# citibeth/spsparse

Hardware: AMD Instinct MI355X
Metric: nnz(C)/s for C=A*A SpGEMM (higher is better)
Workload: dtype f64

## Files before the change

### spsparse_amd/csrc/capi.hip

```cpp
#include "internal.h"

#include <cstdio>
#include <cstdlib>
#include <cstring>
#include <algorithm>
#include <exception>
#include <vector>

using namespace spsamd;

#define API_GUARD(ctx, ...)                                                         \
	if ((ctx)->busy) { (ctx)->last_error = "context busy: a streamed multiply is delivering on it"; return SPSAMD_EINVAL; } \
	try { __VA_ARGS__ }                                                             \
	catch (const spsamd::Error &e) { (ctx)->last_error = e.msg; return e.code; }    \
	catch (const std::bad_alloc &) { (ctx)->last_error = "host allocation failed"; return SPSAMD_ENOMEM; } \
	catch (const std::exception &e) { (ctx)->last_error = e.what(); return SPSAMD_EINVAL; }

extern "C" const char *spsamd_version(void) { return "spsparse_amd 0.2 (gfx950)"; }

extern "C" int spsamd_ctx_create(spsamd_ctx **out, int device, void *hip_stream)
{
	if (!out) return SPSAMD_EINVAL;
	*out = nullptr;
	int ndev = 0;
// ... 223 lines not shown
			SPS_HIP(hipMemcpyAsync(vv, V->val, V->nnz * sizeof(double), kind, c->stream));
			fill_zero(c, vz, V->nnz * sizeof(int32_t));
			Vm.idx0 = vi; Vm.idx1 = vz; Vm.val = vv;
		}
		int rc = multiply_body(c, C, scalei, A, transpose_A, scalej, &Vm, '.', nullptr, duplicate_policy, zero_nan,
			sink_kind, sink_flags & ~SPSAMD_SINK_PERMUTE, res, "V", true, nullptr, true);
		res->shape1 = 0;
		res->idx1 = nullptr;
		return rc;
	)
}


struct spsamd_operand {
	spsamd::Prepared p;
	uint64_t shape0 = 0, shape1 = 0;
};

extern "C" int spsamd_operand_prepare(spsamd_ctx *c, const spsamd_coo *X, char transpose, int role, int duplicate_policy, int zero_nan,
	spsamd_operand **out)
{
	if (!c) return SPSAMD_EINVAL;
	API_GUARD(c,
		if (!X || !out) throw Error{SPSAMD_EINVAL, "null operand or result"};
		*out = nullptr;
		if (role != SPSAMD_AS_A && role != SPSAMD_AS_B && role != (SPSAMD_AS_A | SPSAMD_AS_B)) throw Error{SPSAMD_EINVAL, "bad role"};
		if (duplicate_policy < 0 || duplicate_policy > 2) throw Error{SPSAMD_EINVAL, "bad duplicate_policy"};
		if (X->mem == SPSAMD_MEM_PREPARED) throw Error{SPSAMD_EINVAL, "the operand is a prepared one already"};
		if (zero_nan && role == (SPSAMD_AS_A | SPSAMD_AS_B))
			throw Error{SPSAMD_EINVAL, "under zero_nan the two sides of a product drop different NaNs (multiply_sparse.hpp:167-168): prepare one operand per side"};
		SPS_HIP(hipSetDevice(c->device));
		c->arena.reset();
		const int lead = transpose == 'T' ? 1 : 0;
		const int ref_lead = (role & SPSAMD_AS_A) ? lead : 1 - lead;
		ConMat m;
		consolidate_operand(c, X, lead, ref_lead, duplicate_policy, zero_nan, &m);
		spsamd_operand *h = new spsamd_operand();
		struct Guard { spsamd_operand *h; ~Guard() { if (h) { h->p.release(); delete h; } } } guard{h};
		h->shape0 = X->shape0; h->shape1 = X->shape1;
		Prepared &p = h->p;
		p.ctx = c; p.owns = true; p.lead = lead;
		p.m = m;
		const size_t n = m.nnz;
		size_t want = (n + 64) * (16 + 12 + 8) + (m.nrow + 66) * 4 + 65536;
		uint32_t maxlen = 0;
		if (n) {
			Prepared view;
			view.ctx = c; view.m = m;
			prepared_row_structure(c, &view);
			maxlen = view.maxlen;
		}
		if ((role & SPSAMD_AS_B) && maxlen > 64) {
			const uint64_t W = m.ncol > (uint64_t(1) << 21) ? 16384 : 8192, nwin = (m.ncol + W - 1) / W, nwp = (nwin + 7) & ~7ull, nrowb = m.nrow + 1;
			const uint64_t idx = nrowb * (nwin + 1) * 4 + nrowb * nwp * 2 + (nrowb * nwin + 1) * 4 + (n + 8) * 12 + 8192;
			size_t freeb = 0, totalb = 0;
			if (idx <= 64 * (uint64_t)n * 16 && hipMemGetInfo(&freeb, &totalb) == hipSuccess && idx + want < freeb / 2) want += idx;
		}
		p.reserve(want);
		p.m.row = p.get<int32_t>(n ? n : 1); p.m.col = p.get<int32_t>(n ? n : 1); p.m.val = p.get<double>(n ? n : 1);
		if (n) {
			SPS_HIP(hipMemcpyAsync(p.m.row, m.row, n * sizeof(int32_t), hipMemcpyDeviceToDevice, c->stream));
			SPS_HIP(hipMemcpyAsync(p.m.col, m.col, n * sizeof(int32_t), hipMemcpyDeviceToDevice, c->stream));
			SPS_HIP(hipMemcpyAsync(p.m.val, m.val, n * sizeof(double), hipMemcpyDeviceToDevice, c->stream));
		}
		prepared_row_structure(c, &p);
		SPS_HIP(hipStreamSynchronize(c->stream));
		guard.h = nullptr;
		*out = h;
		return SPSAMD_OK;
	)
}

extern "C" int spsamd_operand_as_coo(const spsamd_operand *h, spsamd_coo *out)
{
	if (!h || !out) return SPSAMD_EINVAL;
	out->idx0 = (const int32_t *)h; out->idx1 = nullptr; out->val = nullptr;
	out->nnz = h->p.m.nnz; out->shape0 = h->shape0; out->shape1 = h->shape1;
	out->sort0 = h->p.lead; out->mem = SPSAMD_MEM_PREPARED;
	return SPSAMD_OK;
}

extern "C" uint64_t spsamd_operand_bytes(const spsamd_operand *h) { return h ? h->p.owned_bytes : 0; }

extern "C" void spsamd_operand_destroy(spsamd_operand *h)
{
	if (!h) return;
	if (h->p.ctx) { (void)hipSetDevice(h->p.ctx->device); (void)hipStreamSynchronize(h->p.ctx->stream); if (h->p.ctx->side) (void)hipStreamSynchronize(h->p.ctx->side); }
	h->p.release();
	delete h;
}

extern "C" int spsamd_result_fetch(spsamd_ctx *c, const spsamd_result *res, spsamd_chunk_fn cb, void *user)
{
	if (!c) return SPSAMD_EINVAL;
	API_GUARD(c,
		if (!res || !cb) throw Error{SPSAMD_EINVAL, "null result or callback"};
		if (res->nnz == 0) return SPSAMD_OK;
		if (!res->idx0 || !res->val) throw Error{SPSAMD_EINVAL, "result has no COO tuples (DIGEST sink?)"};
		SPS_HIP(hipSetDevice(c->device));
		const size_t chunk = size_t(1) << 20;
		char *h = (char *)c->host_staging(2 * chunk * 16);
		hipEvent_t ev[2] = {c->ev[EV_FETCH0], c->ev[EV_FETCH1]};
		auto issue = [&](uint64_t o, int b) {
			size_t n = (size_t)std::min<uint64_t>(chunk, res->nnz - o);
			char *hb = h + (size_t)b * chunk * 16;
			SPS_HIP(hipMemcpyAsync(hb, res->idx0 + o, n * 4, hipMemcpyDeviceToHost, c->stream));
			if (res->idx1) SPS_HIP(hipMemcpyAsync(hb + chunk * 4, res->idx1 + o, n * 4, hipMemcpyDeviceToHost, c->stream));
// ... 315 lines not shown
```

### spsparse_amd/csrc/internal.h

```cpp
#pragma once

#include <hip/hip_runtime.h>
#include <stdint.h>
#include <stddef.h>
#include <string>
#include <vector>

#include "../../include/spsparse_amd.h"

namespace spsamd {


struct Error {
	int code;
	std::string msg;
};

#define SPS_HIP(call)                                                              \
	do {                                                                           \
		hipError_t e_ = (call);                                                    \
		if (e_ != hipSuccess)                                                      \
			throw ::spsamd::Error{SPSAMD_EHIP, std::string(#call) + ": " + hipGetErrorString(e_)}; \
	} while (0)

// ... 264 lines not shown

void first_kept_key_raw(spsamd_ctx *c, const spsamd_coo *Xdev, int lead, int ref_lead, unsigned long long *out_dev);

uint32_t inspect_operand(spsamd_ctx *c, const int32_t *major, const int32_t *minor, const double *val, size_t n,
	uint64_t nrow, uint64_t ncol);

struct RowList {
	uint32_t *beg = nullptr;
	int32_t *id = nullptr;
	uint32_t nrows = 0;
};
void dim_beginnings(spsamd_ctx *c, const ConMat &m, RowList *out);
void dim_beginnings(spsamd_ctx *c, const ConMat &m, const uint32_t *ptr, RowList *out);

uint32_t *sorted_permutation(spsamd_ctx *c, const spsamd_coo *X, int lead);

uint32_t *dense_rowptr(spsamd_ctx *c, const ConMat &m, uint32_t extra, uint32_t *into = nullptr);

struct __attribute__((packed, aligned(4))) BTup { int32_t col; uint32_t vlo, vhi; };

struct SolveSchedule {
	bool built = false;
	uint32_t levels = 0, max_level_rows = 0;
	uint64_t tuples_used = 0;
	int64_t zero_pivot = -1;
	uint32_t *level_ptr = nullptr;
	uint32_t *rows = nullptr;
	std::vector<uint32_t> h_level_ptr, h_level_max;
	bool have_work = false;
	std::vector<uint32_t> h_level_work;
};

struct Prepared {
	spsamd_ctx *ctx = nullptr;
	ConMat m;
	int lead = 0;
	bool owns = false;
	std::vector<void *> owned;
	uint64_t owned_bytes = 0;
	char *slab = nullptr;
	size_t slab_left = 0;
	void reserve(size_t bytes);
	uint32_t *rowptr = nullptr;
	uint32_t maxlen = 0;
	bool have_maxlen = false;
	RowList rl;
	bool have_rl = false;
	BTup *btup = nullptr;
	int W = 0;
	uint32_t nwin = 0, nwp = 0;
	uint64_t nrowb = 0;
	uint32_t *bwin = nullptr;
	uint16_t *wcnt = nullptr;
	uint32_t *wptr = nullptr;
	BTup *btw = nullptr;
	SolveSchedule solve[2][2];
	void *alloc(size_t bytes);
	template <class T> T *get(size_t n) { return (T *)alloc(n * sizeof(T)); }
	void release();
};


struct ScaleDev {
	bool present = false;
	int32_t *pos = nullptr;
	const double *val = nullptr;
	uint64_t dim = 0;
};

void upload_scale(spsamd_ctx *c, const spsamd_vec *s, uint64_t dim, const char *name, ScaleDev *out);

struct MultiplyArgs {
	double C;
	ScaleDev si, sj, sk;
	ConMat A, B;
	int sink_kind, sink_flags;
	Prepared *pa = nullptr, *pb = nullptr;
	hipEvent_t b_ready = nullptr;
	OutSet *out = nullptr;
	bool static_walk = false;
};
void spgemm(spsamd_ctx *c, MultiplyArgs &a, spsamd_result *res);
void prepared_row_structure(spsamd_ctx *c, Prepared *p);
BTup *prepared_btup(spsamd_ctx *c, Prepared *p);

struct OperandParts { Prepared *pa = nullptr, *pb = nullptr; hipEvent_t b_ready = nullptr; };
int multiply_body(spsamd_ctx *c, double C,
	const spsamd_vec *scalei, const spsamd_coo *A, char transpose_A,
	const spsamd_vec *scalej, const spsamd_coo *B, char transpose_B,
	const spsamd_vec *scalek, int duplicate_policy, int zero_nan,
	int sink_kind, int sink_flags, spsamd_result *res, const char *what, bool arena_ready, const OperandParts *parts = nullptr, bool b_rank1 = false);


int multiply_stream(spsamd_ctx *c, double C,
	const spsamd_vec *scalei, const spsamd_coo *A, char transpose_A,
	const spsamd_vec *scalej, const spsamd_coo *B, char transpose_B,
	const spsamd_vec *scalek, int duplicate_policy, int zero_nan,
	int sink_flags, size_t block_tuples, spsamd_chunk_fn cb, void *user,
	spsamd_result *res, spsamd_stream_stats *stats);


struct DenseOperand {
	const uint32_t *rowptr = nullptr;
	const BTup *tup = nullptr;
	uint64_t nrow = 0, ncol = 0;
	uint32_t nnz = 0;
// ... 155 lines not shown
```

### spsparse_amd/csrc/k_hash.hip

```cpp
#include "spgemm_host.h"
#include "spgemm_hash.h"

namespace spsamd {

template <int T, int NT, int MODE, bool WINDOWED, bool PAT>
__global__ __launch_bounds__(NT) void k_hash(const Cell *cells, uint32_t ncell, const uint32_t *xb, RowMeta m,
	const uint32_t *bwin, uint32_t nwin1, EmitParams ep, SinkParams sk)
{
	__shared__ int32_t h_key[T];
	__shared__ double h_val[MODE == MODE_COUNT ? 1 : T];
	__shared__ uint16_t occ[T / 2];
	__shared__ uint64_t s_sort[MODE == MODE_STORE ? T / 2 : 1];
	__shared__ uint16_t s_cnt[MODE == MODE_STORE ? 16 * ((T / 2 + NT - 1) / NT) * (NT / 64) : 1];
	__shared__ Expand<NT, T / 2> X;
	__shared__ uint32_t scr32[NT / 64 + 1];
	__shared__ uint32_t s_nocc;
	__shared__ PatCell s_pat;
	__shared__ unsigned long long s_u64[2 * (NT / 64)];
	__shared__ double s_f64[NT / 64];

	const unsigned tid = threadIdx.x;
	for (int q = tid; q < T; q += NT) { h_key[q] = -1; if (MODE != MODE_COUNT) h_val[q] = 0.0; }
	PatAcc pat; pat_init(pat);
	if (tid == 0) pat_reset(&s_pat);
	DigestAcc dacc{0, 0, 0.0};
	uint32_t flip = 0;

	const CellWalk walk = cell_walk(xb, ncell);
	const uint32_t stride = walk.stride, cend = walk.end;
	const bool any_cell = walk.first < cend;
	const uint32_t clast = any_cell ? cend - 1 : 0;
	const uint32_t zlane = cell_pend_zero();
	Cell rec1 = cells[min(walk.first, clast)];
	CellPend pend2 = cell_pend_load(cells, min(walk.first + stride, clast), zlane);
	uint32_t nlo, nlen; double na;
	{
		const uint32_t e = rec1.beg + tid;
		const bool act = e < rec1.end;
		const uint32_t ec = act ? e : rec1.beg;
		const int32_t k = m.acol[ec];
		uint32_t lo, hi;
		if (WINDOWED) { const uint32_t *bw = bwin + (uint64_t)k * nwin1; lo = bw[rec1.wa]; hi = bw[rec1.wb]; }
		else { lo = m.bptr[k]; hi = m.bptr[k + 1]; }
		na = m.aval[ec];
		nlo = lo; nlen = act ? hi - lo : 0u;
	}
	for (uint32_t ci = walk.first; ci < cend; ci += stride) {
		const Cell cell = rec1;
		const uint32_t beg = cell.beg, end = cell.end, wa = cell.wa, wb = cell.wb, seg = cell.seg;
		const int32_t rowid = cell.rowid;
		const uint32_t lo0 = nlo, len0 = nlen; const double a0 = na;
		rec1 = cell_from_pend(pend2);
		pend2 = cell_pend_load(cells, min(ci + 2 * stride, clast), zlane);
		const uint32_t ne = rec1.beg + tid;
		const bool nact = (ci + stride < cend) && ne < rec1.end;
		const uint32_t nec = ne < rec1.end ? ne : rec1.beg;
		const int32_t nk = m.acol[nec];
		na = m.aval[nec];
		const bool oversize = cell.prods > (uint32_t)(T / 2);
		if (oversize && tid == 0) atomicOr(sk.err, 1u);
		lds_barrier();
		if (tid == 0) s_nocc = 0;

		for (uint32_t chunk = beg; chunk < (oversize ? beg : end); chunk += NT) {
			uint32_t lo = lo0, len = len0; double a = a0;
			if (chunk != beg) {
				uint32_t e = chunk + tid;
				lo = 0; len = 0; a = 0;
				if (e < end) {
					int32_t k = m.acol[e];
					if (WINDOWED) { const uint32_t *bw = bwin + (uint64_t)k * nwin1; lo = bw[wa]; len = bw[wb] - lo; }
					else { lo = m.bptr[k]; len = m.bptr[k + 1] - lo; }
					a = m.aval[e];
				}
			}
			uint32_t total, nzc, ex;
			expand_load(X, lo, len, a, &total, &nzc, flip, &ex);
			if (total == 0) continue;
			if (!ABL(ep, 4)) expand_batch(X, 0, total, nzc);
			if (ABL(ep, 1)) total = 0;
			if (ep.ordered) hash_products_ordered<T, NT, T / 2, MODE>(X, 0, nzc, m, h_key, h_val, occ, &s_nocc);
			else hash_products<T, NT, T / 2, MODE, PAT>(X, 0, total, 0, m, h_key, h_val, occ, &s_nocc, pat);
			lds_barrier();
		}
		if (PAT) pat_publish(pat, &s_pat);
		{
			uint32_t lo, hi;
			if (WINDOWED) { const uint32_t *bw = bwin + (uint64_t)nk * nwin1; lo = bw[rec1.wa]; hi = bw[rec1.wb]; }
			else { lo = m.bptr[nk]; hi = m.bptr[nk + 1]; }
			nlo = lo; nlen = nact ? hi - lo : 0u;
		}
		lds_barrier();
		uint32_t nocc = s_nocc;
		if (ABL(ep, 2)) nocc = 0;
		uint32_t colbase = 0, colbits = ep.ncolbits;
		if (WINDOWED) { colbase = wa << ep.wshift; colbits = ep.wshift + (wb - wa > 1 ? 32 - __builtin_clz(wb - wa - 1) : 0); }
		const double pthr = PAT ? pat_threshold(&s_pat, end - beg) : -1.0;
		hash_emit<T, NT, MODE, PAT>(nocc, rowid, seg, ep, sk, h_key, h_val, occ, s_sort, scr32, dacc, s_cnt, colbase, colbits, m, beg, end, pthr);
		if (PAT) { lds_barrier(); if (tid == 0) pat_reset(&s_pat); }
	}
	if (MODE == MODE_DIGEST) digest_flush<NT>(sk.digest, dacc.cnt, dacc.hash, dacc.sum, s_u64, s_f64);
}

template <int MODE>
__global__ __launch_bounds__(TILE_NT) void k_hash_tiles(const Tile *tiles, uint32_t ntile, const TCell *tcells, RowMeta m,
	const uint32_t *bwin, uint32_t nwin1, EmitParams ep, SinkParams sk)
{
	constexpr int NT = TILE_NT, T = TILE_T;
	__shared__ int32_t h_key[T];
	__shared__ double h_val[MODE == MODE_COUNT ? 1 : T];
	__shared__ uint16_t occ[T / 2];
	__shared__ uint64_t s_sort[MODE == MODE_STORE ? T / 2 : 1];
	__shared__ uint16_t s_cnt[MODE == MODE_STORE ? 16 * ((T / 2 + NT - 1) / NT) * (NT / 64) : 1];
	constexpr int PB = MODE == MODE_STORE ? TILE_PB_STORE : TILE_PB;
	__shared__ Expand<NT, PB> X;
	__shared__ uint32_t scr32[NT / 64 + 1];
	__shared__ uint32_t s_nocc;
	__shared__ PatCell s_pat;
	__shared__ uint32_t cellP[TILE_MAXCELLS + 1];
	__shared__ unsigned long long s_u64[2 * (NT / 64)];
	__shared__ double s_f64[NT / 64];

	const unsigned tid = threadIdx.x;
	for (int q = tid; q < T; q += NT) { h_key[q] = -1; if (MODE != MODE_COUNT) h_val[q] = 0.0; }
	PatAcc pat; pat_init(pat);
	if (tid == 0) pat_reset(&s_pat);
	DigestAcc dacc{0, 0, 0.0};
	uint32_t flip = 0;
	STAMP_BEGIN();
	TileWalk<BoundsRowMajor, false> walk;
	for (walk.begin(tiles, ntile, tcells, m.acol, m.aval, BoundsRowMajor{bwin, nwin1}); walk.more(); walk.next()) {
		const TileTake t = walk.take();
		const Tile &tile = t.tile;
		const uint32_t myc = tid >> t.lsh, myei = tid & ((1u << t.lsh) - 1u);

		STAMP_COUNT(8);
		STAMP(0);
		lds_barrier();
		STAMP(1);
		uint32_t total, nzc, ex;
		expand_load(X, t.lo, t.len, t.a, &total, &nzc, flip, &ex);
		if (myei == 0 && myc < tile.ncells) cellP[myc] = ex;
		if (tid == 0) { cellP[tile.ncells] = total; s_nocc = 0; }
		const uint32_t seg_of_mine = t.seg;
		STAMP(2);
		if (total) expand_batch(X, 0, total, nzc);
		else lds_barrier();
		STAMP(3);
		walk.expanded();
		for (uint32_t c = 0; c < tile.ncells; ++c) {
			STAMP_COUNT(9);
			STAMP(0);
			const uint32_t p0 = cellP[c], p1 = cellP[c + 1];
			if (ep.ordered) {
				const uint32_t q0 = expand_lookup(X, p0, 0), q1 = expand_lookup(X, p1 - 1, 0) + 1;
				hash_products_ordered<T, NT, PB, MODE>(X, q0, q1, m, h_key, h_val, occ, &s_nocc);
			} else if (ep.pattern) hash_products<T, NT, PB, MODE, true>(X, p0, p1, 0, m, h_key, h_val, occ, &s_nocc, pat);
			else hash_products<T, NT, PB, MODE, false>(X, p0, p1, 0, m, h_key, h_val, occ, &s_nocc, pat);
			if (ep.pattern) pat_publish(pat, &s_pat);
			STAMP(4);
			lds_barrier();
			STAMP(5);
			const uint32_t nocc = s_nocc;
			if (myc == c && myei == 0) scr32[NT / 64] = seg_of_mine;
			lds_barrier();
			const uint32_t seg = scr32[NT / 64];
			if (tid == 0) s_nocc = 0;
			uint32_t colbase = 0, colbits = 0;
			if (MODE == MODE_STORE) {
				const TCell tcc = tcells[tile.first + c];
				colbase = (uint32_t)tcc.wa << ep.wshift;
				colbits = ep.wshift + (tcc.wb - tcc.wa > 1 ? 32 - __builtin_clz((uint32_t)(tcc.wb - tcc.wa) - 1u) : 0);
			}
			STAMP(6);
			const double pthr = ep.pattern ? pat_threshold(&s_pat, tile.end - tile.beg) : -1.0;
			if (ep.pattern) hash_emit<T, NT, MODE, true>(nocc, tile.rowid, seg, ep, sk, h_key, h_val, occ, s_sort, scr32, dacc, s_cnt, colbase, colbits, m, tile.beg, tile.end, pthr);
			else hash_emit<T, NT, MODE, false>(nocc, tile.rowid, seg, ep, sk, h_key, h_val, occ, s_sort, scr32, dacc, s_cnt, colbase, colbits, m, tile.beg, tile.end, pthr);
			STAMP(7);
			if (ep.pattern) { lds_barrier(); if (tid == 0) pat_reset(&s_pat); }
			lds_barrier();
		}
	}
	STAMP_FLUSH();
	if (MODE == MODE_DIGEST) digest_flush<NT>(sk.digest, dacc.cnt, dacc.hash, dacc.sum, s_u64, s_f64);
}

template <int T, int NT, int MODE, bool WINDOWED>
static void launch_hash(spsamd_ctx *c, const Cell *cells, uint32_t ncell, const uint32_t *xb, const RowMeta &m, const uint32_t *bwin,
	uint32_t nwin1, const EmitParams &ep, const SinkParams &sk)
{
	if (!ncell) return;
	unsigned grid = std::min<unsigned>(ncell, (unsigned)(c->num_cu * resident_per_cu<&k_hash<T, NT, MODE, WINDOWED, false>>(NT)));
	if (grid >= 64) grid &= ~7u;
	if (ep.pattern) k_hash<T, NT, MODE, WINDOWED, true><<<dim3(grid), dim3(NT), 0, c->stream>>>(cells, ncell, xb, m, bwin, nwin1, ep, sk);
	else k_hash<T, NT, MODE, WINDOWED, false><<<dim3(grid), dim3(NT), 0, c->stream>>>(cells, ncell, xb, m, bwin, nwin1, ep, sk);
	SPS_LAUNCH_CHECK();
}

template <int MODE>
void launch_mid(spsamd_ctx *c, const Bins &b, const MidCells &mc, const RowMeta &m, const EmitParams &ep, const SinkParams &sk)
{
	launch_hash<1024, 256, MODE, false>(c, mc.cells[0], b.count[5], nullptr, m, nullptr, 0, ep, sk);
	launch_hash<4096, 512, MODE, false>(c, mc.cells[1], b.count[6], nullptr, m, nullptr, 0, ep, sk);
	launch_hash<8192, 512, MODE, false>(c, mc.cells[2], b.count[7], nullptr, m, nullptr, 0, ep, sk);
}

template <int MODE>
void launch_hash_windowed(spsamd_ctx *c, const Heavy &hv, const RowMeta &m, const EmitParams &ep, const SinkParams &sk)
{
	launch_hash<1024, 256, MODE, true>(c, hv.cells[0], hv.ncell[0], hv.xb[0], m, hv.bwin, hv.nwin1, ep, sk);
	launch_hash<3072, 512, MODE, true>(c, hv.cells[1], hv.ncell[1], hv.xb[1], m, hv.bwin, hv.nwin1, ep, sk);
	launch_hash<4096, 512, MODE, true>(c, hv.cells[2], hv.ncell[2], hv.xb[2], m, hv.bwin, hv.nwin1, ep, sk);
	launch_hash<8192, 512, MODE, true>(c, hv.cells[3], hv.ncell[3], hv.xb[3], m, hv.bwin, hv.nwin1, ep, sk);
}

template <int MODE>
void launch_tiles_v1(spsamd_ctx *c, const Heavy &hv, const RowMeta &m, const EmitParams &ep, const SinkParams &sk)
{
	const unsigned grid = std::min<unsigned>(hv.ntile, (unsigned)(c->num_cu * resident_per_cu<&k_hash_tiles<MODE>>(TILE_NT)));
	const SinkParams &sks = stamps_sink(c, sk, grid);
	k_hash_tiles<MODE><<<dim3(grid), dim3(TILE_NT), 0, c->stream>>>(hv.tb.tiles, hv.ntile, hv.tb.tcells, m, hv.bwin, hv.nwin1, ep, sks);
	SPS_LAUNCH_CHECK();
	static const char *const nm[10] = {"pre", "Bwait", "expand_load", "expand_batch", "products", "Bwait2", "segbcast", "emit", "tiles", "cells"};
	stamps_report(c, sks, grid, "k_hash_tiles", nm, 10);
}

template void launch_mid<MODE_COUNT>(spsamd_ctx *, const Bins &, const MidCells &, const RowMeta &, const EmitParams &, const SinkParams &);
template void launch_mid<MODE_STORE>(spsamd_ctx *, const Bins &, const MidCells &, const RowMeta &, const EmitParams &, const SinkParams &);
template void launch_mid<MODE_DIGEST>(spsamd_ctx *, const Bins &, const MidCells &, const RowMeta &, const EmitParams &, const SinkParams &);
template void launch_hash_windowed<MODE_COUNT>(spsamd_ctx *, const Heavy &, const RowMeta &, const EmitParams &, const SinkParams &);
template void launch_hash_windowed<MODE_STORE>(spsamd_ctx *, const Heavy &, const RowMeta &, const EmitParams &, const SinkParams &);
template void launch_hash_windowed<MODE_DIGEST>(spsamd_ctx *, const Heavy &, const RowMeta &, const EmitParams &, const SinkParams &);
template void launch_tiles_v1<MODE_COUNT>(spsamd_ctx *, const Heavy &, const RowMeta &, const EmitParams &, const SinkParams &);
template void launch_tiles_v1<MODE_STORE>(spsamd_ctx *, const Heavy &, const RowMeta &, const EmitParams &, const SinkParams &);
template void launch_tiles_v1<MODE_DIGEST>(spsamd_ctx *, const Heavy &, const RowMeta &, const EmitParams &, const SinkParams &);

#ifdef SPSAMD_ABLATIONS
void set_ablation_word(spsamd_ctx *c, int word)
{
	SPS_HIP(hipMemcpyToSymbolAsync(HIP_SYMBOL(g_abl), &word, sizeof(int), 0, hipMemcpyHostToDevice, c->stream));
	SPS_HIP(hipStreamSynchronize(c->stream));
}
#endif

}
```

### spsparse_amd/csrc/spgemm_host.h

```cpp
#pragma once
#include "spgemm_dev.h"

namespace spsamd {

struct Bins {
	uint32_t count[NBIN];
	uint32_t off[NBIN + 1];
	uint32_t *rows;
};

struct MidCells { Cell *cells[3] = {nullptr, nullptr, nullptr}; };

struct TooWide { uint64_t width; };
constexpr uint64_t COLBLK = (uint64_t)2048 << 14;

struct Heavy {
	uint32_t n = 0;
	uint64_t tuples = 0;
	uint32_t *rows = nullptr;
	uint32_t *bwin = nullptr;
	uint32_t nwin = 0, nwin1 = 0;
	uint32_t *winprod = nullptr;
	uint32_t ncell[NCLS] = {};
	Cell *cells[NCLS] = {};
	CellBases cnt{}, base{};
	uint32_t *xb[NCLS] = {};
	int W = 8192;
	uint32_t cell_cap = CELL_CAP_DEFAULT, dense_min = DENSE_MIN_DEFAULT;
	TileBases tb{};
	uint32_t ntile = 0, ntcell = 0;
	TileBases tb2{};
	uint32_t ntile2 = 0, ntcell2 = 0;
	uint32_t direct_min = 0;
	int tiles2 = 0;
	uint32_t *tile_ctr = nullptr;
	uint32_t span_cap = 0;
	uint32_t alt_cap = 0, alt_span = 0;
	unsigned long long *alt_cells = nullptr;
	uint32_t long_cap = 0, long_dense_min = 0;
	bool coo = false;
	unsigned long long clsprod[NCLS + 2] = {};
	uint32_t *wptr = nullptr;
	BTup *btw = nullptr;
	uint64_t nrowb = 0;
	uint32_t nnzb = 0;

	uint32_t narrow() const { return ((uint64_t)nnzb + DENSE_R) * 12u < (uint64_t(1) << 32) ? 1u : 0u; }
	template <int MODE> uint32_t *tile_claim() const { return tile_ctr ? tile_ctr + (MODE == MODE_STORE ? 1 : 0) : nullptr; }
};

static inline TileKinds tile_kinds(const Heavy &hv)
{
	TileKinds tk{{hv.tb, hv.tb2}, hv.direct_min, hv.span_cap, hv.long_cap, hv.long_dense_min,
		hv.tiles2 == 0 ? (uint32_t)BM_MAXOUT : (uint32_t)(TILE_T / 2), hv.alt_cap, hv.alt_span, hv.alt_cells};
	return tk;
}

static inline float elapsed(hipEvent_t a, hipEvent_t b)
{
	float ms = 0;
	SPS_HIP(hipEventElapsedTime(&ms, a, b));
	return ms;
}

template <auto KERNEL>
static inline int resident_per_cu(int nt)
{
	static int per_cu = 0;
	if (!per_cu) {
		int nb = 0;
		if (hipOccupancyMaxActiveBlocksPerMultiprocessor(&nb, KERNEL, nt, 0) != hipSuccess || nb < 1) nb = 1;
		per_cu = nb;
	}
// ... 62 lines not shown
```

### spsparse_amd/csrc/symbolic_heavy.hip

```cpp
#include "spgemm_host.h"

namespace spsamd {

__global__ void k_cell_cost(const Cell *cells, uint32_t n, uint32_t fixed, uint32_t *cost)
{
	uint32_t i = blockIdx.x * blockDim.x + threadIdx.x;
	if (i < n) cost[i] = cells[i].prods + fixed;
}

__global__ void k_xcd_bounds(const int64_t *pref, uint32_t n, uint32_t *xb)
{
	uint32_t x = threadIdx.x;
	if (x > 8) return;
	int64_t target = pref[n] / 8 * x;
	uint32_t lo = 0, hi = n;
	while (lo < hi) { uint32_t mid = lo + ((hi - lo) >> 1); if (pref[mid] < target) lo = mid + 1; else hi = mid; }
	xb[x] = x == 8 ? n : lo;
}


constexpr int BT_NT = 256;
constexpr size_t BT_LDS = 36 * 1024;

__global__ __launch_bounds__(BT_NT) void k_wcnt_count(const int32_t *brow, const int32_t *bcol, uint32_t nnzb, uint32_t wshift, uint32_t nwp, uint32_t *wcnt32)
{
	const uint32_t lane = lane_id();
	const uint32_t nchunk = (nnzb + 63u) >> 6, nwaves = gridDim.x * (BT_NT / 64);
	for (uint32_t ch = blockIdx.x * (BT_NT / 64) + wave_id(); ch < nchunk; ch += nwaves) {
		const uint32_t e = (ch << 6) + lane;
		const bool valid = e < nnzb;
		const unsigned long long key = valid ? (unsigned long long)(uint32_t)brow[e] * nwp + ((uint32_t)bcol[e] >> wshift) : ~0ull;
		const unsigned long long kprev = __shfl_up(key, 1, 64), knext = __shfl_down(key, 1, 64);
		const bool is_start = valid && (lane == 0 || key != kprev);
		const bool is_end = valid && (lane == 63 || key != knext);
		const unsigned long long sm = __ballot(is_start);
		if (is_end) {
			const unsigned long long upto = sm & (lane == 63 ? ~0ull : ((2ull << lane) - 1ull));
			const uint32_t first = 63u - (uint32_t)__clzll((long long)upto);
			atomicAdd(&wcnt32[key >> 1], (lane - first + 1u) << ((uint32_t)(key & 1ull) << 4));
		}
	}
}

__global__ __launch_bounds__(BT_NT) void k_bwin_scan(const uint16_t *wcnt, const uint32_t *bptr, uint64_t nrowb, uint32_t tr, uint32_t nwin, uint32_t nwp,
	uint32_t *bwin)
{
	extern __shared__ uint32_t s_dyn[];
	const uint32_t nwin1 = nwin + 1u, lane = lane_id(), wv = wave_id(), nph = nwp >> 1;
	const uint64_t k0 = (uint64_t)blockIdx.x * tr;
	const uint32_t rows = (uint32_t)std::min<uint64_t>(tr, nrowb - k0);
	uint32_t *s_ptr = s_dyn + (size_t)tr * nph;
	{
		const uint4 *src = reinterpret_cast<const uint4 *>(wcnt + k0 * nwp);
		uint4 *dst = reinterpret_cast<uint4 *>(s_dyn);
		for (uint32_t i = threadIdx.x; i < (rows * nph) >> 2; i += BT_NT) dst[i] = src[i];
		for (uint32_t r = threadIdx.x; r < rows; r += BT_NT) s_ptr[r] = bptr[k0 + r];
	}
	__syncthreads();
	for (uint32_t r = wv; r < rows; r += BT_NT / 64) {
		const uint32_t *src = s_dyn + r * nph;
		uint32_t carry = s_ptr[r];
		uint32_t *bw = bwin + (k0 + r) * nwin1;
		for (uint32_t c0 = 0; c0 < nwin1; c0 += 64u) {
			const uint32_t w = c0 + lane;
			const uint32_t v = w < nwin ? (src[w >> 1] >> ((w & 1u) << 4)) & 0xFFFFu : 0u;
			const uint32_t inc = wave_inclusive_scan_u32(v);
			if (w < nwin1) bw[w] = carry + inc - v;
			carry += (uint32_t)__builtin_amdgcn_readlane((int)inc, 63);
		}
	}
}

constexpr int WM_TR = 256;
constexpr int WM_CS = 72;
constexpr int WM_NT = 256;

__global__ __launch_bounds__(WM_NT) void k_wm_tile_sums(const uint16_t *wcnt, uint64_t nrowb, uint32_t nwp, uint32_t ntile, uint32_t *tilesum)
{
	extern __shared__ uint32_t s_dyn[];
	const uint32_t nq = nwp >> 3;
	for (uint32_t w = threadIdx.x; w < nwp; w += WM_NT) s_dyn[w] = 0;
	__syncthreads();
	const uint64_t k0 = (uint64_t)blockIdx.x * WM_TR;
	const uint32_t rows = (uint32_t)std::min<uint64_t>(WM_TR, nrowb - k0);
	const uint4 *tab = reinterpret_cast<const uint4 *>(wcnt + k0 * nwp);
	uint32_t acc[8] = {0, 0, 0, 0, 0, 0, 0, 0};
	uint32_t myq = 0xFFFFFFFFu;
	const uint32_t stride = (WM_NT / nq) * nq;
	if (threadIdx.x < stride) {
		myq = threadIdx.x % nq;
		for (uint32_t i = threadIdx.x; i < rows * nq; i += stride) {
			const uint4 x = tab[i];
			acc[0] += x.x & 0xFFFFu; acc[1] += x.x >> 16; acc[2] += x.y & 0xFFFFu; acc[3] += x.y >> 16;
			acc[4] += x.z & 0xFFFFu; acc[5] += x.z >> 16; acc[6] += x.w & 0xFFFFu; acc[7] += x.w >> 16;
		}
#pragma unroll
		for (int u = 0; u < 8; ++u) if (acc[u]) atomicAdd(&s_dyn[myq * 8u + u], acc[u]);
	}
	__syncthreads();
	for (uint32_t w = threadIdx.x; w < nwp; w += WM_NT) tilesum[(uint64_t)w * ntile + blockIdx.x] = s_dyn[w];
}

__global__ __launch_bounds__(WM_NT) void k_wm_tile_scan(uint32_t *tilesum, uint32_t ntile, uint32_t *wtot)
{
	__shared__ uint32_t scratch[WM_NT / 64 + 1];
	uint32_t *a = tilesum + (uint64_t)blockIdx.x * ntile;
	uint32_t carry = 0;
	for (uint32_t base = 0; base < ntile; base += WM_NT) {
		const uint32_t i = base + threadIdx.x;
		const uint32_t v = i < ntile ? a[i] : 0u;
		uint32_t tot;
		const uint32_t ex = block_exclusive_scan<uint32_t, WM_NT>(v, scratch, &tot);
		if (i < ntile) a[i] = carry + ex;
		carry += tot;
	}
	if (threadIdx.x == 0) wtot[blockIdx.x] = carry;
}

// ... 269 lines not shown
{
	uint32_t i = blockIdx.x * blockDim.x + threadIdx.x;
	if (i < n) dst[i] = src[perm[i]];
}

static void heavy_window_major(spsamd_ctx *c, Heavy &hv, const ConMat &B, uint32_t wshift, const uint16_t *wcnt, uint32_t nwp, Prepared *pb)
{
	hipStream_t st = c->stream;
	const uint64_t nrowb = hv.nrowb, total = nrowb * hv.nwin;
	const uint32_t ntile = (uint32_t)((nrowb + WM_TR - 1) / WM_TR);
	hv.wptr = pb->get<uint32_t>(total + 1);
	uint32_t *tilesum = c->arena.get<uint32_t>((uint64_t)nwp * ntile);
	uint32_t *wtot = c->arena.get<uint32_t>(hv.nwin), *wbase = c->arena.get<uint32_t>(hv.nwin);
	k_wm_tile_sums<<<dim3(ntile), dim3(WM_NT), nwp * sizeof(uint32_t), st>>>(wcnt, nrowb, nwp, ntile, tilesum);
	SPS_LAUNCH_CHECK();
	k_wm_tile_scan<<<dim3(hv.nwin), dim3(WM_NT), 0, st>>>(tilesum, ntile, wtot);
	SPS_LAUNCH_CHECK();
	k_wm_bases<<<dim3(1), dim3(WM_NT), 0, st>>>(wtot, hv.nwin, wbase, hv.wptr + total);
	SPS_LAUNCH_CHECK();
	k_wm_ptr<<<dim3(ntile), dim3(WM_NT), 0, st>>>(wcnt, nrowb, hv.nwin, nwp, ntile, tilesum, wbase, hv.wptr);
	SPS_LAUNCH_CHECK();
	hv.btw = pb->get<BTup>((size_t)B.nnz + DENSE_R);
	k_wm_scatter<<<dim3(grid_for(B.nnz)), dim3(256), 0, st>>>(B.row, B.col, B.val, B.nnz, wshift, hv.bwin, hv.nwin1, hv.wptr, nrowb, hv.btw);
	SPS_LAUNCH_CHECK();
}

int heavy_b_index(spsamd_ctx *c, const ConMat &B, const uint32_t *bptr, uint32_t extra, uint64_t nheavy, Prepared *pb)
{
	hipStream_t st = c->stream;
	int W = B.ncol > (uint64_t(1) << 21) ? 16384 : 8192;
	if (c->tune.window == 8192 || c->tune.window == 16384) W = c->tune.window;
	const uint32_t wshift = W == 8192 ? 13 : 14;
	const uint32_t nwin = (uint32_t)((B.ncol + W - 1) >> wshift);
	if (nwin > (uint32_t)WH_MAXW) throw TooWide{COLBLK};
	const uint64_t nrowb = B.nrow + extra;
	if (pb->bwin && pb->W == W && pb->nrowb == nrowb) return W;
	const uint64_t per_window = nrowb * 12u + nheavy * 4u;
	uint64_t budget;
	const uint64_t room = (pb->owns || c->arena.slabs.empty()) ? 0 : c->arena.slabs.back().cap - c->arena.slabs.back().used;
	if (c->tune.index_budget_mb > 0) budget = (uint64_t)c->tune.index_budget_mb << 20;
	else if (per_window * (nwin + 1ull) <= room) budget = room;
	else {
		size_t freeb = 0, totalb = 0;
		SPS_HIP(hipMemGetInfo(&freeb, &totalb));
		budget = (uint64_t)((double)(freeb + room) * 0.8);
	}
	if (per_window * (nwin + 1ull) > budget && nwin > 1) {
		uint64_t fit = budget / per_window;
		if (fit < 2) throw Error{SPSAMD_ENOMEM, "the window index of one column window of op(B) does not fit the device"};
		uint64_t w2 = 1;
		while (w2 * 2 <= fit - 1) w2 *= 2;
		throw TooWide{w2 << wshift};
	}
	const uint32_t nwin1 = nwin + 1, nwp = (nwin + 7u) & ~7u;
	pb->reserve(nrowb * nwin1 * 4 + nrowb * nwp * 2 + (nrowb * nwin + 1) * 4 + ((size_t)B.nnz + DENSE_R) * sizeof(BTup) + 4096);
	pb->bwin = pb->get<uint32_t>(nrowb * nwin1);
	pb->wcnt = pb->get<uint16_t>(nrowb * nwp);
	pb->W = W; pb->nwin = nwin; pb->nwp = nwp; pb->nrowb = nrowb;
	pb->wptr = nullptr; pb->btw = nullptr;
	fill_zero(c, pb->wcnt, nrowb * nwp * sizeof(uint16_t));
	k_wcnt_count<<<dim3((unsigned)c->num_cu * 16u), dim3(BT_NT), 0, st>>>(B.row, B.col, B.nnz, wshift, nwp, reinterpret_cast<uint32_t *>(pb->wcnt));
	SPS_LAUNCH_CHECK();
	uint32_t tr = 256;
	while (tr > 4 && (size_t)tr * (nwp * 2 + 4) > BT_LDS) tr >>= 1;
	static bool lds_attr = false;
	if (!lds_attr) { SPS_HIP(hipFuncSetAttribute((const void *)k_bwin_scan, hipFuncAttributeMaxDynamicSharedMemorySize, (int)BT_LDS)); lds_attr = true; }
	k_bwin_scan<<<dim3((unsigned)((nrowb + tr - 1) / tr)), dim3(BT_NT), (size_t)tr * (nwp * 2 + 4), st>>>(pb->wcnt, bptr, nrowb, tr, nwin, nwp, pb->bwin);
	SPS_LAUNCH_CHECK();
	return W;
}

void heavy_prepare(spsamd_ctx *c, Heavy &hv, const Bins &bins, const RowMeta &m, const ConMat &B, const uint32_t *bptr,
	uint32_t extra, uint32_t *nseg, bool ordered, bool pattern, Prepared *pb)
{
	hipStream_t st = c->stream;
	hv.W = heavy_b_index(c, B, bptr, extra, hv.n, pb);
	const uint32_t wshift = hv.W == 8192 ? 13 : 14;
	hv.nwin = (uint32_t)((B.ncol + hv.W - 1) >> wshift);
	hv.nwin1 = hv.nwin + 1;
	const uint64_t nrowb = B.nrow + extra;
	const bool have_wmajor = pb->wptr != nullptr;
	hv.nrowb = nrowb;
	hv.nnzb = B.nnz;
	hv.rows = bins.rows + bins.off[8];
	hv.winprod = c->arena.get<uint32_t>((uint64_t)hv.n * hv.nwin);
	const uint32_t nwp = (hv.nwin + 7u) & ~7u;
	hv.bwin = pb->bwin;
	uint16_t *wcnt = pb->wcnt;
	if (!c->tune.no_wmajor && have_wmajor) { hv.wptr = pb->wptr; hv.btw = pb->btw; }
	else if (!c->tune.no_wmajor) {
		{
			SideScope on_side(c, 0, true);
			heavy_window_major(c, hv, B, wshift, wcnt, nwp, pb);
		}
		pb->wptr = hv.wptr; pb->btw = hv.btw;
	}
	uint32_t *hubcount = c->arena.get<uint32_t>(1);
	const uint32_t hubcap = (uint32_t)(hv.tuples / WH_PART) + 1u;
	HubItem *hublist = c->arena.get<HubItem>(hubcap);
	fill_zero(c, hubcount, sizeof(uint32_t));
	k_win_hist<<<dim3(hv.n), dim3(WH_NT), 0, st>>>(hv.rows, hv.n, m, wcnt, hv.nwin, nwp, hv.winprod, hubcount, hublist, hubcap);
	SPS_LAUNCH_CHECK();
	k_win_hist_hub<<<dim3((unsigned)c->num_cu * 8u), dim3(WH_NT), 0, st>>>(hv.rows, m, wcnt, hv.nwin, nwp, hv.winprod, hubcount, hublist, hubcap);
	SPS_LAUNCH_CHECK();
	for (int k = 0; k < NCLS; ++k) {
		hv.cnt.base[k] = c->arena.get<uint32_t>(hv.n);
		hv.base.base[k] = c->arena.get<uint32_t>((size_t)hv.n + 1);
	}
	if (c->tune.cell_cap >= 64 && c->tune.cell_cap <= (int)CELL_CAP) hv.cell_cap = (uint32_t)c->tune.cell_cap;
	if (c->tune.dense_min >= 64 && c->tune.dense_min <= (int)CELL_CAP) hv.dense_min = (uint32_t)c->tune.dense_min;
	const size_t hn4 = ((size_t)hv.n + 3) & ~(size_t)3;
	uint32_t *zblock = c->arena.get<uint32_t>(4 * hn4 + 2 * (NCLS + 2) + 4 + 2);
	const size_t zbytes = (4 * hn4 + 2 * (NCLS + 2) + 4 + 2) * sizeof(uint32_t);
	unsigned long long *clsprod = reinterpret_cast<unsigned long long *>(zblock + 4 * hn4);
	unsigned long long *alt_block = clsprod + NCLS + 2;
	hv.tile_ctr = c->tune.tile_walk == 1 ? nullptr : zblock + 4 * hn4 + 2 * (NCLS + 2) + 4;
	hv.tb.enabled = !c->tune.no_tiles;
	const bool free_choice = !ordered && c->tune.tiles_v1 == 0;
	const bool user_dense_min = c->tune.dense_min >= 64 && c->tune.dense_min <= (int)CELL_CAP;
	auto set_scheme = [&](int scheme) {
		hv.tiles2 = scheme;
		if (!user_dense_min) hv.dense_min = scheme == 0 && hv.tb.enabled ? DENSE_MIN_BITMAP : DENSE_MIN_DEFAULT;
		hv.tb.by_items = scheme != 1 ? 1 : 0;
		hv.tb.pb = scheme != 1 ? (uint32_t)TILE2_ITEMS : (hv.coo ? (uint32_t)TILE_PB_STORE : (uint32_t)TILE_PB);
		hv.span_cap = scheme == 0 ? (uint32_t)BM_WORDS >> (wshift - 6) : 0u;
	};
	set_scheme(ordered ? 1 : (c->tune.tiles_v1 == 1 ? (pattern ? 2 : 1) : (c->tune.tiles_v1 == 2 ? 2 : 0)));
	hv.long_dense_min = c->tune.long_dense_min > 0 ? (uint32_t)c->tune.long_dense_min : (hv.W == 8192 ? LONG_DENSE_MIN_DEFAULT : 0u);
	hv.long_cap = c->tune.long_cap > 0 ? (uint32_t)std::min<int>(c->tune.long_cap, (int)CELL_CAP) : 0u;
	hv.tb2.by_items = 1;
	hv.direct_min = c->tune.direct_min > 0 ? (uint32_t)c->tune.direct_min : DIRECT_MIN_DEFAULT;
	hv.tb2.enabled = hv.tb.enabled && !c->tune.no_wmajor && !ordered && !pattern && hv.direct_min < hv.dense_min;
	hv.tb2.pb = (uint32_t)hv.W;
	{
		int q = 0;
		for (TileBases *t : {&hv.tb, &hv.tb2}) {
			t->ntc = zblock + hn4 * q++; t->ntl = zblock + hn4 * q++;
			t->tcbase = c->arena.get<uint32_t>((size_t)hv.n + 1); t->tlbase = c->arena.get<uint32_t>((size_t)hv.n + 1);
		}
	}
// ... 115 lines not shown
```

Baseline: 163.0 billion.

## Skip empty B-row windows in windowed hash via occupancy bitmap and LDS queue

Result: faster. 165.9 billion, median of 6 (+1.8%).

```diff
diff --git a/spsparse_amd/csrc/capi.hip b/spsparse_amd/csrc/capi.hip
--- a/spsparse_amd/csrc/capi.hip
+++ b/spsparse_amd/csrc/capi.hip
@@ -299,7 +299,8 @@
 		}
 		if ((role & SPSAMD_AS_B) && maxlen > 64) {
 			const uint64_t W = m.ncol > (uint64_t(1) << 21) ? 16384 : 8192, nwin = (m.ncol + W - 1) / W, nwp = (nwin + 7) & ~7ull, nrowb = m.nrow + 1;
-			const uint64_t idx = nrowb * (nwin + 1) * 4 + nrowb * nwp * 2 + (nrowb * nwin + 1) * 4 + (n + 8) * 12 + 8192;
+			const uint64_t nbw = (((nwin + 31) >> 5) + 3) & ~3ull;
+			const uint64_t idx = nrowb * (nwin + 1) * 4 + nrowb * nwp * 2 + nrowb * nbw * 4 + (nrowb * nwin + 1) * 4 + (n + 8) * 12 + 8192;
 			size_t freeb = 0, totalb = 0;
 			if (idx <= 64 * (uint64_t)n * 16 && hipMemGetInfo(&freeb, &totalb) == hipSuccess && idx + want < freeb / 2) want += idx;
 		}
diff --git a/spsparse_amd/csrc/internal.h b/spsparse_amd/csrc/internal.h
--- a/spsparse_amd/csrc/internal.h
+++ b/spsparse_amd/csrc/internal.h
@@ -340,6 +340,8 @@
 	uint64_t nrowb = 0;
 	uint32_t *bwin = nullptr;
 	uint16_t *wcnt = nullptr;
+	uint32_t *bocc = nullptr;
+	uint32_t nbw = 0;
 	uint32_t *wptr = nullptr;
 	BTup *btw = nullptr;
 	SolveSchedule solve[2][2];
diff --git a/spsparse_amd/csrc/k_hash.hip b/spsparse_amd/csrc/k_hash.hip
--- a/spsparse_amd/csrc/k_hash.hip
+++ b/spsparse_amd/csrc/k_hash.hip
@@ -3,9 +3,32 @@
 
 namespace spsamd {
 
+__device__ __forceinline__ uint4 bocc_load(const uint32_t *bocc, uint32_t nbw, uint32_t k, uint32_t g)
+{
+	return reinterpret_cast<const uint4 *>(bocc + (uint64_t)k * nbw)[g];
+}
+__device__ __forceinline__ uint32_t bocc_word_mask(uint32_t lo, uint32_t hi, uint32_t base)
+{
+	const uint32_t a = lo > base ? min(lo - base, 32u) : 0u, b = hi > base ? min(hi - base, 32u) : 0u;
+	return (uint32_t)(((1ull << b) - 1ull) & ~((1ull << a) - 1ull));
+}
+__device__ __forceinline__ uint32_t bocc_test(const uint4 &x, uint32_t g, uint32_t wa, uint32_t wb)
+{
+	const uint32_t b0 = g << 7, lo = max(wa, b0) - b0, hi = min(wb, b0 + 128u) - b0;
+	return (x.x & bocc_word_mask(lo, hi, 0)) | (x.y & bocc_word_mask(lo, hi, 32)) | (x.z & bocc_word_mask(lo, hi, 64)) | (x.w & bocc_word_mask(lo, hi, 96));
+}
+__device__ __forceinline__ uint32_t bocc_rest(const uint32_t *bocc, uint32_t nbw, uint32_t k, uint32_t g0, uint32_t wa, uint32_t wb)
+{
+	uint32_t bits = 0;
+	for (uint32_t g = g0 + 1u; g <= (wb - 1u) >> 7; ++g) bits |= bocc_test(bocc_load(bocc, nbw, k, g), g, wa, wb);
+	return bits;
+}
+
+constexpr int long_steps(int T, int MODE) { return T == 1024 ? (MODE == MODE_STORE ? 1 : 3) : (T == 3072 ? 2 : (T == 4096 ? 3 : 4)); }
+
 template <int T, int NT, int MODE, bool WINDOWED, bool PAT>
 __global__ __launch_bounds__(NT) void k_hash(const Cell *cells, uint32_t ncell, const uint32_t *xb, RowMeta m,
-	const uint32_t *bwin, uint32_t nwin1, EmitParams ep, SinkParams sk)
+	const uint32_t *bwin, uint32_t nwin1, EmitParams ep, SinkParams sk, const uint32_t *bocc, uint32_t nbw)
 {
 	__shared__ int32_t h_key[T];
 	__shared__ double h_val[MODE == MODE_COUNT ? 1 : T];
@@ -18,6 +41,8 @@
 	__shared__ PatCell s_pat;
 	__shared__ unsigned long long s_u64[2 * (NT / 64)];
 	__shared__ double s_f64[NT / 64];
+	__shared__ uint2 s_queue[WINDOWED && MODE != MODE_STORE ? NT * (long_steps(T, MODE) + 1) : 1];
+	__shared__ uint32_t s_qcnt[2][NT / 64];
 
 	const unsigned tid = threadIdx.x;
 	for (int q = tid; q < T; q += NT) { h_key[q] = -1; if (MODE != MODE_COUNT) h_val[q] = 0.0; }
@@ -33,21 +58,20 @@
 	const uint32_t zlane = cell_pend_zero();
 	Cell rec1 = cells[min(walk.first, clast)];
 	CellPend pend2 = cell_pend_load(cells, min(walk.first + stride, clast), zlane);
+	if constexpr (!WINDOWED) {
 	uint32_t nlo, nlen; double na;
 	{
 		const uint32_t e = rec1.beg + tid;
 		const bool act = e < rec1.end;
 		const uint32_t ec = act ? e : rec1.beg;
 		const int32_t k = m.acol[ec];
-		uint32_t lo, hi;
-		if (WINDOWED) { const uint32_t *bw = bwin + (uint64_t)k * nwin1; lo = bw[rec1.wa]; hi = bw[rec1.wb]; }
-		else { lo = m.bptr[k]; hi = m.bptr[k + 1]; }
+		const uint32_t lo = m.bptr[k], hi = m.bptr[k + 1];
 		na = m.aval[ec];
 		nlo = lo; nlen = act ? hi - lo : 0u;
 	}
 	for (uint32_t ci = walk.first; ci < cend; ci += stride) {
 		const Cell cell = rec1;
-		const uint32_t beg = cell.beg, end = cell.end, wa = cell.wa, wb = cell.wb, seg = cell.seg;
+		const uint32_t beg = cell.beg, end = cell.end, seg = cell.seg;
 		const int32_t rowid = cell.rowid;
 		const uint32_t lo0 = nlo, len0 = nlen; const double a0 = na;
 		rec1 = cell_from_pend(pend2);
@@ -69,8 +93,7 @@
 				lo = 0; len = 0; a = 0;
 				if (e < end) {
 					int32_t k = m.acol[e];
-					if (WINDOWED) { const uint32_t *bw = bwin + (uint64_t)k * nwin1; lo = bw[wa]; len = bw[wb] - lo; }
-					else { lo = m.bptr[k]; len = m.bptr[k + 1] - lo; }
+					lo = m.bptr[k]; len = m.bptr[k + 1] - lo;
 					a = m.aval[e];
 				}
 			}
@@ -85,19 +108,116 @@
 		}
 		if (PAT) pat_publish(pat, &s_pat);
 		{
-			uint32_t lo, hi;
-			if (WINDOWED) { const uint32_t *bw = bwin + (uint64_t)nk * nwin1; lo = bw[rec1.wa]; hi = bw[rec1.wb]; }
-			else { lo = m.bptr[nk]; hi = m.bptr[nk + 1]; }
+			const uint32_t lo = m.bptr[nk], hi = m.bptr[nk + 1];
 			nlo = lo; nlen = nact ? hi - lo : 0u;
 		}
 		lds_barrier();
 		uint32_t nocc = s_nocc;
 		if (ABL(ep, 2)) nocc = 0;
-		uint32_t colbase = 0, colbits = ep.ncolbits;
-		if (WINDOWED) { colbase = wa << ep.wshift; colbits = ep.wshift + (wb - wa > 1 ? 32 - __builtin_clz(wb - wa - 1) : 0); }
+		const double pthr = PAT ? pat_threshold(&s_pat, end - beg) : -1.0;
+		hash_emit<T, NT, MODE, PAT>(nocc, rowid, seg, ep, sk, h_key, h_val, occ, s_sort, scr32, dacc, s_cnt, 0, ep.ncolbits, m, beg, end, pthr);
+		if (PAT) { lds_barrier(); if (tid == 0) pat_reset(&s_pat); }
+	}
+	} else {
+	constexpr int NW = NT / 64, U = long_steps(T, MODE);
+	constexpr uint32_t QCAP = (uint32_t)NT * (U + 1);
+	static_assert(MODE != MODE_STORE || QCAP <= (uint32_t)(T / 2), "the ring fits s_sort");
+	uint2 *const queue = MODE == MODE_STORE ? reinterpret_cast<uint2 *>(s_sort) : s_queue;
+	const uint32_t lane = lane_id(), wv = wave_id();
+	const uint32_t mypos = (wv * U) * 64u + lane;
+	uint32_t qflip = 0;
+	int32_t nk[U];
+#pragma unroll
+	for (int u = 0; u < U; ++u) { const uint32_t e = rec1.beg + mypos + u * 64u; nk[u] = m.acol[e < rec1.end ? e : rec1.beg]; }
+	for (uint32_t ci = walk.first; ci < cend; ci += stride) {
+		const Cell cell = rec1;
+		const uint32_t beg = cell.beg, end = cell.end, wa = cell.wa, wb = cell.wb, seg = cell.seg, g0 = wa >> 7;
+		const int32_t rowid = cell.rowid;
+		int32_t k0[U];
+#pragma unroll
+		for (int u = 0; u < U; ++u) k0[u] = nk[u];
+		rec1 = cell_from_pend(pend2);
+		pend2 = cell_pend_load(cells, min(ci + 2 * stride, clast), zlane);
+#pragma unroll
+		for (int u = 0; u < U; ++u) { const uint32_t e = rec1.beg + mypos + u * 64u; nk[u] = m.acol[e < rec1.end ? e : rec1.beg]; }
+		const bool oversize = cell.prods > (uint32_t)(T / 2);
+		if (oversize && tid == 0) atomicOr(sk.err, 1u);
+		lds_barrier();
+		if (tid == 0) s_nocc = 0;
+
+		const uint32_t stop = oversize ? beg : end;
+		uint32_t pos = beg, qh = 0, qt = 0, qn = 0;
+		while (pos < stop || qn) {
+			if (pos < stop && qn < (uint32_t)NT) {
+				int32_t kk[U]; uint4 x[U];
+				if (pos == beg) {
+#pragma unroll
+					for (int u = 0; u < U; ++u) kk[u] = k0[u];
+				} else {
+#pragma unroll
+					for (int u = 0; u < U; ++u) { const uint32_t e = pos + mypos + u * 64u; kk[u] = m.acol[e < end ? e : beg]; }
+				}
+#pragma unroll
+				for (int u = 0; u < U; ++u) x[u] = bocc_load(bocc, nbw, (uint32_t)kk[u], g0);
+				unsigned long long bm[U]; uint32_t wt = 0;
+#pragma unroll
+				for (int u = 0; u < U; ++u) {
+					const uint32_t bits = bocc_test(x[u], g0, wa, wb) | bocc_rest(bocc, nbw, (uint32_t)kk[u], g0, wa, wb);
+					bm[u] = __ballot(pos + mypos + u * 64u < end && bits != 0u);
+					wt += (uint32_t)__popcll(bm[u]);
+				}
+				if (lane == 0) s_qcnt[qflip][wv] = wt;
+				lds_barrier();
+				uint32_t off = qt, tot = 0;
+#pragma unroll
+				for (int w = 0; w < NW; ++w) { const uint32_t c = s_qcnt[qflip][w]; if (w < (int)wv) off += c; tot += c; }
+				qflip ^= 1u;
+				tot = (uint32_t)__builtin_amdgcn_readfirstlane((int)tot);
+#pragma unroll
+				for (int u = 0; u < U; ++u) {
+					if ((bm[u] >> lane) & 1ull) {
+						uint32_t idx = off + (uint32_t)__popcll(bm[u] & lanemask_lt());
+						if (idx >= QCAP) idx -= QCAP;
+						queue[idx] = make_uint2(pos + mypos + u * 64u, (uint32_t)kk[u]);
+					}
+					off += (uint32_t)__popcll(bm[u]);
+				}
+				qt += tot; if (qt >= QCAP) qt -= QCAP;
+				qn += tot;
+				pos += (uint32_t)NT * U;
+				lds_barrier();
+				continue;
+			}
+			const uint32_t n = min(qn, (uint32_t)NT);
+			uint32_t lo = 0, len = 0; double a = 0;
+			if (tid < n) {
+				uint32_t idx = qh + tid;
+				if (idx >= QCAP) idx -= QCAP;
+				const uint2 q = queue[idx];
+				const uint32_t *bw = bwin + (uint64_t)q.y * nwin1;
+				lo = bw[wa]; len = bw[wb] - lo;
+				a = m.aval[q.x];
+			}
+			qh += n; if (qh >= QCAP) qh -= QCAP;
+			qn -= n;
+			uint32_t total, nzc, ex;
+			expand_load(X, lo, len, a, &total, &nzc, flip, &ex);
+			if (total == 0) continue;
+			if (!ABL(ep, 4)) expand_batch(X, 0, total, nzc);
+			if (ABL(ep, 1)) total = 0;
+			if (ep.ordered) hash_products_ordered<T, NT, T / 2, MODE>(X, 0, nzc, m, h_key, h_val, occ, &s_nocc);
+			else hash_products<T, NT, T / 2, MODE, PAT>(X, 0, total, 0, m, h_key, h_val, occ, &s_nocc, pat);
+			lds_barrier();
+		}
+		if (PAT) pat_publish(pat, &s_pat);
+		lds_barrier();
+		uint32_t nocc = s_nocc;
+		if (ABL(ep, 2)) nocc = 0;
+		const uint32_t colbase = wa << ep.wshift, colbits = ep.wshift + (wb - wa > 1 ? 32 - __builtin_clz(wb - wa - 1) : 0);
 		const double pthr = PAT ? pat_threshold(&s_pat, end - beg) : -1.0;
 		hash_emit<T, NT, MODE, PAT>(nocc, rowid, seg, ep, sk, h_key, h_val, occ, s_sort, scr32, dacc, s_cnt, colbase, colbits, m, beg, end, pthr);
 		if (PAT) { lds_barrier(); if (tid == 0) pat_reset(&s_pat); }
+	}
 	}
 	if (MODE == MODE_DIGEST) digest_flush<NT>(sk.digest, dacc.cnt, dacc.hash, dacc.sum, s_u64, s_f64);
 }
@@ -187,13 +307,13 @@
 
 template <int T, int NT, int MODE, bool WINDOWED>
 static void launch_hash(spsamd_ctx *c, const Cell *cells, uint32_t ncell, const uint32_t *xb, const RowMeta &m, const uint32_t *bwin,
-	uint32_t nwin1, const EmitParams &ep, const SinkParams &sk)
+	uint32_t nwin1, const EmitParams &ep, const SinkParams &sk, const uint32_t *bocc = nullptr, uint32_t nbw = 0)
 {
 	if (!ncell) return;
 	unsigned grid = std::min<unsigned>(ncell, (unsigned)(c->num_cu * resident_per_cu<&k_hash<T, NT, MODE, WINDOWED, false>>(NT)));
 	if (grid >= 64) grid &= ~7u;
-	if (ep.pattern) k_hash<T, NT, MODE, WINDOWED, true><<<dim3(grid), dim3(NT), 0, c->stream>>>(cells, ncell, xb, m, bwin, nwin1, ep, sk);
-	else k_hash<T, NT, MODE, WINDOWED, false><<<dim3(grid), dim3(NT), 0, c->stream>>>(cells, ncell, xb, m, bwin, nwin1, ep, sk);
+	if (ep.pattern) k_hash<T, NT, MODE, WINDOWED, true><<<dim3(grid), dim3(NT), 0, c->stream>>>(cells, ncell, xb, m, bwin, nwin1, ep, sk, bocc, nbw);
+	else k_hash<T, NT, MODE, WINDOWED, false><<<dim3(grid), dim3(NT), 0, c->stream>>>(cells, ncell, xb, m, bwin, nwin1, ep, sk, bocc, nbw);
 	SPS_LAUNCH_CHECK();
 }
 
@@ -208,10 +328,10 @@
 template <int MODE>
 void launch_hash_windowed(spsamd_ctx *c, const Heavy &hv, const RowMeta &m, const EmitParams &ep, const SinkParams &sk)
 {
-	launch_hash<1024, 256, MODE, true>(c, hv.cells[0], hv.ncell[0], hv.xb[0], m, hv.bwin, hv.nwin1, ep, sk);
-	launch_hash<3072, 512, MODE, true>(c, hv.cells[1], hv.ncell[1], hv.xb[1], m, hv.bwin, hv.nwin1, ep, sk);
-	launch_hash<4096, 512, MODE, true>(c, hv.cells[2], hv.ncell[2], hv.xb[2], m, hv.bwin, hv.nwin1, ep, sk);
-	launch_hash<8192, 512, MODE, true>(c, hv.cells[3], hv.ncell[3], hv.xb[3], m, hv.bwin, hv.nwin1, ep, sk);
+	launch_hash<1024, 256, MODE, true>(c, hv.cells[0], hv.ncell[0], hv.xb[0], m, hv.bwin, hv.nwin1, ep, sk, hv.bocc, hv.nbw);
+	launch_hash<3072, 512, MODE, true>(c, hv.cells[1], hv.ncell[1], hv.xb[1], m, hv.bwin, hv.nwin1, ep, sk, hv.bocc, hv.nbw);
+	launch_hash<4096, 512, MODE, true>(c, hv.cells[2], hv.ncell[2], hv.xb[2], m, hv.bwin, hv.nwin1, ep, sk, hv.bocc, hv.nbw);
+	launch_hash<8192, 512, MODE, true>(c, hv.cells[3], hv.ncell[3], hv.xb[3], m, hv.bwin, hv.nwin1, ep, sk, hv.bocc, hv.nbw);
 }
 
 template <int MODE>
diff --git a/spsparse_amd/csrc/spgemm_host.h b/spsparse_amd/csrc/spgemm_host.h
--- a/spsparse_amd/csrc/spgemm_host.h
+++ b/spsparse_amd/csrc/spgemm_host.h
@@ -19,6 +19,8 @@
 	uint64_t tuples = 0;
 	uint32_t *rows = nullptr;
 	uint32_t *bwin = nullptr;
+	uint32_t *bocc = nullptr;
+	uint32_t nbw = 0;
 	uint32_t nwin = 0, nwin1 = 0;
 	uint32_t *winprod = nullptr;
 	uint32_t ncell[NCLS] = {};
diff --git a/spsparse_amd/csrc/symbolic_heavy.hip b/spsparse_amd/csrc/symbolic_heavy.hip
--- a/spsparse_amd/csrc/symbolic_heavy.hip
+++ b/spsparse_amd/csrc/symbolic_heavy.hip
@@ -43,7 +43,7 @@
 }
 
 __global__ __launch_bounds__(BT_NT) void k_bwin_scan(const uint16_t *wcnt, const uint32_t *bptr, uint64_t nrowb, uint32_t tr, uint32_t nwin, uint32_t nwp,
-	uint32_t *bwin)
+	uint32_t *bwin, uint32_t *bocc, uint32_t nbw)
 {
 	extern __shared__ uint32_t s_dyn[];
 	const uint32_t nwin1 = nwin + 1u, lane = lane_id(), wv = wave_id(), nph = nwp >> 1;
@@ -61,9 +61,13 @@
 		const uint32_t *src = s_dyn + r * nph;
 		uint32_t carry = s_ptr[r];
 		uint32_t *bw = bwin + (k0 + r) * nwin1;
-		for (uint32_t c0 = 0; c0 < nwin1; c0 += 64u) {
+		uint32_t *bo = bocc + (k0 + r) * nbw;
+		const uint32_t cend = max(nwin1, nbw << 5);
+		for (uint32_t c0 = 0; c0 < cend; c0 += 64u) {
 			const uint32_t w = c0 + lane;
 			const uint32_t v = w < nwin ? (src[w >> 1] >> ((w & 1u) << 4)) & 0xFFFFu : 0u;
+			const unsigned long long nz = __ballot(v != 0u);
+			if (lane < 2u && (c0 >> 5) + lane < nbw) bo[(c0 >> 5) + lane] = (uint32_t)(nz >> (lane << 5));
 			const uint32_t inc = wave_inclusive_scan_u32(v);
 			if (w < nwin1) bw[w] = carry + inc - v;
 			carry += (uint32_t)__builtin_amdgcn_readlane((int)inc, 63);
@@ -439,11 +443,12 @@
 		while (w2 * 2 <= fit - 1) w2 *= 2;
 		throw TooWide{w2 << wshift};
 	}
-	const uint32_t nwin1 = nwin + 1, nwp = (nwin + 7u) & ~7u;
-	pb->reserve(nrowb * nwin1 * 4 + nrowb * nwp * 2 + (nrowb * nwin + 1) * 4 + ((size_t)B.nnz + DENSE_R) * sizeof(BTup) + 4096);
+	const uint32_t nwin1 = nwin + 1, nwp = (nwin + 7u) & ~7u, nbw = (((nwin + 31u) >> 5) + 3u) & ~3u;
+	pb->reserve(nrowb * nwin1 * 4 + nrowb * nwp * 2 + nrowb * nbw * 4 + (nrowb * nwin + 1) * 4 + ((size_t)B.nnz + DENSE_R) * sizeof(BTup) + 4096);
 	pb->bwin = pb->get<uint32_t>(nrowb * nwin1);
 	pb->wcnt = pb->get<uint16_t>(nrowb * nwp);
-	pb->W = W; pb->nwin = nwin; pb->nwp = nwp; pb->nrowb = nrowb;
+	pb->bocc = pb->get<uint32_t>(nrowb * nbw);
+	pb->W = W; pb->nwin = nwin; pb->nwp = nwp; pb->nbw = nbw; pb->nrowb = nrowb;
 	pb->wptr = nullptr; pb->btw = nullptr;
 	fill_zero(c, pb->wcnt, nrowb * nwp * sizeof(uint16_t));
 	k_wcnt_count<<<dim3((unsigned)c->num_cu * 16u), dim3(BT_NT), 0, st>>>(B.row, B.col, B.nnz, wshift, nwp, reinterpret_cast<uint32_t *>(pb->wcnt));
@@ -452,7 +457,7 @@
 	while (tr > 4 && (size_t)tr * (nwp * 2 + 4) > BT_LDS) tr >>= 1;
 	static bool lds_attr = false;
 	if (!lds_attr) { SPS_HIP(hipFuncSetAttribute((const void *)k_bwin_scan, hipFuncAttributeMaxDynamicSharedMemorySize, (int)BT_LDS)); lds_attr = true; }
-	k_bwin_scan<<<dim3((unsigned)((nrowb + tr - 1) / tr)), dim3(BT_NT), (size_t)tr * (nwp * 2 + 4), st>>>(pb->wcnt, bptr, nrowb, tr, nwin, nwp, pb->bwin);
+	k_bwin_scan<<<dim3((unsigned)((nrowb + tr - 1) / tr)), dim3(BT_NT), (size_t)tr * (nwp * 2 + 4), st>>>(pb->wcnt, bptr, nrowb, tr, nwin, nwp, pb->bwin, pb->bocc, nbw);
 	SPS_LAUNCH_CHECK();
 	return W;
 }
@@ -473,6 +478,7 @@
 	hv.winprod = c->arena.get<uint32_t>((uint64_t)hv.n * hv.nwin);
 	const uint32_t nwp = (hv.nwin + 7u) & ~7u;
 	hv.bwin = pb->bwin;
+	hv.bocc = pb->bocc; hv.nbw = pb->nbw;
 	uint16_t *wcnt = pb->wcnt;
 	if (!c->tune.no_wmajor && have_wmajor) { hv.wptr = pb->wptr; hv.btw = pb->btw; }
 	else if (!c->tune.no_wmajor) {
```
